# baegwangbin/MaGNet

Measured on NVIDIA H100. Metric: frames/sec (640x480, 4 views, 64 hyp), higher is better.
Workload: dtype f32

## Files before the change

magnet_b200/csrc/cost_mma.cu:

```cuda
#include <cuda_bf16.h>
#include <cuda_fp16.h>

#include <algorithm>
#include <atomic>
#include <cstddef>
#include <mutex>
#include <type_traits>

#include "common.cuh"
#include "tma_common.cuh"
#include "cw_mask.cuh"

namespace magnet {

constexpr int MNT = 256;
constexpr int MTW = 8, MTH = 8;
constexpr int MPX = MTW * MTH;
constexpr int MCH = 64;
constexpr int MSEG = 32;
constexpr int MMAXV = 16;
constexpr int SEG_BYTES = 2048;
constexpr int META_SEG_BYTES = 128;
constexpr uint32_t SEG_TX = 1024;
constexpr uint32_t REF_TX = 8192;

constexpr int MOFF_A = 0;
constexpr int MOFF_R = 16384;
constexpr int MR_BYTES = 67584;
constexpr int MOFF_META = MOFF_R + MR_BYTES;
constexpr int MOFF_CAM = MOFF_META + MSEG * META_SEG_BYTES;
constexpr int MOFF_KS = MOFF_CAM + MMAXV * 64;
constexpr int MOFF_BBOX = MOFF_KS + MCH * 4;
constexpr int MOFF_BAR = MOFF_BBOX + 64;
constexpr int MOFF_DV = MOFF_BAR + 64;
constexpr int MOFF_DEND = MOFF_DV + MPX * 65 * 4;
constexpr int MOFF_PIXR = MOFF_DEND + MPX * 8;
constexpr int MOFF_PIX = MOFF_PIXR + MPX * 32;
constexpr int M_SMEM_USED = MOFF_PIX + 8 * 8 * 32;
constexpr int M_SMEM_TOTAL = M_SMEM_USED + 1024;
static_assert(MR_BYTES >= MSEG * SEG_BYTES && MR_BYTES >= MPX * 264 * 4 && MR_BYTES >= MCH * 65 * 4, "region R");
constexpr int MMA_DBG_OUTSIDE = 16 + MPX * 256;
static_assert(2 * (M_SMEM_TOTAL + 1024) <= 227 * 1024, "two CTAs per SM");

__host__ __device__ inline size_t split16_bytes(size_t N, size_t H, size_t W) {
  return SPLIT16_HEADER + N * H * W * 256 + N * H * (W + 1) * 16;
}
__host__ __device__ inline size_t half16_bytes(size_t N, size_t H, size_t W) {
  return SPLIT16_HEADER + N * H * W * 128 + N * H * (W + 1) * 16;
}

constexpr int MMA_SLOTS = 1024;
__device__ unsigned g_mma_next[MMA_SLOTS];
__device__ unsigned g_mma_done[MMA_SLOTS];

__device__ __forceinline__ float lds_f32(uint32_t a) {
  float v;
  asm volatile("ld.shared.f32 %0, [%1];" : "=f"(v) : "r"(a));
  return v;
}
__device__ __forceinline__ float4 lds_f32x4(uint32_t a) {
  float4 v;
  asm volatile("ld.shared.v4.f32 {%0, %1, %2, %3}, [%4];" : "=f"(v.x), "=f"(v.y), "=f"(v.z), "=f"(v.w) : "r"(a));
  return v;
}
enum { PROF_SETUP, PROF_BOX, PROF_TMA, PROF_MMA, PROF_PHASEC, PROF_EPI, PROF_NSTAGES };
#ifdef MAGNET_MMA_PROFILE
#define MMA_STAGE(s)                                                                                                   \
  do {                                                                                                                 \
    if (tid == 0) {                                                                                                    \
      const long long t_ = clock64();                                                                                  \
      prof_s[s] += t_ - prof_s[7];                                                                                     \
      prof_s[7] = t_;                                                                                                  \
    }                                                                                                                  \
  } while (0)
#else
#define MMA_STAGE(s) do { } while (0)
#endif

template <int MODE, bool CW, int PLANES>
__global__ void __launch_bounds__(MNT, 2)
cost_mma_kernel(const __grid_constant__ CostParams p, const __grid_constant__ CUtensorMap tm_ref,
                const __grid_constant__ CUtensorMap tm_src, const __grid_constant__ CUtensorMap tm_meta, const int nchunks,
                const int n_items, const int slot, float* __restrict__ dbg) {
  extern __shared__ unsigned char smem_raw[];
  const uint32_t raw = smem_u32(smem_raw);
  const uint32_t padb = (1024u - (raw & 1023u)) & 1023u;
  unsigned char* smem = smem_raw + padb;
  const uint32_t sbase = raw + padb;
  const magnet_camera* cams_s = reinterpret_cast<const magnet_camera*>(smem + MOFF_CAM);
  float* ks = reinterpret_cast<float*>(smem + MOFF_KS);
  int* bbox = reinterpret_cast<int*>(smem + MOFF_BBOX);
  float* regR = reinterpret_cast<float*>(smem + MOFF_R);
  const uint32_t bar_tma = sbase + MOFF_BAR, bar_cam = sbase + MOFF_BAR + 24;
  const unsigned FULL = 0xffffffffu;

  const int tid = threadIdx.x, lane = tid & 31, warp = tid >> 5;
#ifdef MAGNET_MMA_PROFILE
  __shared__ long long prof_s[8];
  if (tid < 8) prof_s[tid] = tid == 7 ? clock64() : 0ll;
#endif
  const int H = p.H, W = p.W, HW = p.HW, D = p.D, V = p.V;
  const int tiles_x = (W + MTW - 1) / MTW;
  const int items_per_b = tiles_x * ((H + MTH - 1) / MTH) * nchunks;

  const unsigned char* refbuf = reinterpret_cast<const unsigned char*>(p.ref_feat);
  const unsigned char* srcbuf = reinterpret_cast<const unsigned char*>(p.src_feat);
  const Split16Header* hdr_ref = reinterpret_cast<const Split16Header*>(refbuf);
  const Split16Header* hdr_src = reinterpret_cast<const Split16Header*>(srcbuf);
  volatile int* next_item = reinterpret_cast<volatile int*>(smem + MOFF_BAR + 40);

  if (tid == 0) {
    mbar_init(bar_tma, 1);
    mbar_init(bar_cam, 1);
    fence_mbar_init();
    prefetch_tmap(&tm_ref);
    prefetch_tmap(&tm_src);
    prefetch_tmap(&tm_meta);
  }
  if (tid < 8) bbox[tid] = (tid & 1) ? -(1 << 28) : (1 << 28);
  __syncthreads();
  uint32_t ph_tma = 0, ph_cam = 0;
  int it = 0;
  int cur_b = -1;
  const float xmax = (float)W + 1.0f, ymax = (float)H + 1.0f;
  const float kappa = p.kappa;
  constexpr float BOX_EPS = 0.015625f;
  const float amp_max = 65536.0f / (float)(max(W, H) + 3) - 8.0f;
  const uint32_t g_row0 = sbase + MOFF_R, m_base = sbase + MOFF_META;

  int item = blockIdx.x;
  while (item < n_items) {
  const int b = item / items_per_b;
  const int rem = item - b * items_per_b;
  const int tile = rem / nchunks;
  const int jc = (rem - tile * nchunks) * MCH;
  const int Dc = min(MCH, D - jc);
  const int tx0 = (tile % tiles_x) * MTW, ty0 = (tile / tiles_x) * MTH;

  if (tid == 0) {
    if (b != cur_b) {
      mbar_arrive_expect_tx(bar_cam, (uint32_t)V * 64u);
      bulk_load(sbase + MOFF_CAM, p.cams + (size_t)b * V, (uint32_t)V * 64u, bar_cam);
    }
    tma_load_5d(sbase + MOFF_A, &tm_ref, bar_tma, 0, tx0, ty0, 0, b);
    *next_item = (int)gridDim.x + (int)atomicAdd(&g_mma_next[slot], 1u);
  }
  if (tid < MCH) ks[tid] = MODE != MAGNET_DEPTH_VOLUME ? p.k[min(jc + tid, D - 1)] : 0.0f;
  __syncthreads();

  const int py = ty0 + warp;
  float4* pixr = reinterpret_cast<float4*>(smem + MOFF_PIXR) + warp * 16;
  unsigned livemask;
  {
    float R0, R1, R2, MU = 0.f, SG = 0.f;
    const int px = tx0 + (lane & 7);
    const bool live = px < W && py < H;
    const int n = min(py, H - 1) * W + min(px, W - 1);
    R0 = ldg_f(p.rays + ((size_t)b * 3 + 0) * HW + n);
    R1 = ldg_f(p.rays + ((size_t)b * 3 + 1) * HW + n);
    R2 = ldg_f(p.rays + ((size_t)b * 3 + 2) * HW + n);
    if (MODE == MAGNET_DEPTH_GAUSS) {
      MU = ldg_f(p.ref_gmm + ((size_t)b * 2 + 0) * HW + n);
      SG = ldg_f(p.ref_gmm + ((size_t)b * 2 + 1) * HW + n);
    }
    livemask = __ballot_sync(FULL, live) & 0xffu;
    if (lane < 8) {
      pixr[2 * lane] = make_float4(R0, R1, R2, 0.0f);
      pixr[2 * lane + 1] = make_float4(MU, SG, 0.0f, 0.0f);
    }
    __syncwarp();
  }
  const uint32_t dvw = sbase + MOFF_DV + (uint32_t)(warp * 8 * 65 + lane) * 4u;
  if (MODE == MAGNET_DEPTH_VOLUME) {
    float* dv_s = reinterpret_cast<float*>(smem + MOFF_DV);
    const int pp = tid & 63, y = ty0 + (pp >> 3), x = tx0 + (pp & 7);
    const float* dsrc = p.d_volume + ((size_t)b * D + jc) * HW + (size_t)min(y, H - 1) * W + min(x, W - 1);
#pragma unroll 1
    for (int j0 = tid >> 6; j0 < MCH; j0 += 32) {
      float dl[8];
#pragma unroll
      for (int r = 0; r < 8; ++r) dl[r] = ldg_f(dsrc + (size_t)min(j0 + 4 * r, Dc - 1) * HW);
#pragma unroll
      for (int r = 0; r < 8; ++r) dv_s[pp * 65 + j0 + 4 * r] = dl[r];
    }
    __syncthreads();
#pragma unroll
    for (int i = 0; i < MTW; ++i) {
      const float da = lds_f32(dvw + i * 260), db = lds_f32(dvw + i * 260 + 128);
      float lo = fminf(da, db), hi = fmaxf(da, db);
      const bool fin = __all_sync(FULL, isfinite(da) && isfinite(db));
#pragma unroll
      for (int o = 16; o > 0; o >>= 1) {
        lo = fminf(lo, __shfl_xor_sync(FULL, lo, o));
        hi = fmaxf(hi, __shfl_xor_sync(FULL, hi, o));
      }
      if (lane == i) reinterpret_cast<float2*>(smem + MOFF_DEND)[warp * 8 + i] = fin ? make_float2(lo, hi) : make_float2(NAN, NAN);
    }
    __syncwarp();
  }
  auto depth2 = [&](const int i, const float mu, const float sg) -> float2 {
    if (MODE == MAGNET_DEPTH_VOLUME) return make_float2(lds_f32(dvw + i * 260), lds_f32(dvw + i * 260 + 128));
    const float2 k2 = make_float2(ks[lane], ks[lane + 32]);
    if (MODE == MAGNET_DEPTH_PLANES) return k2;
    return fadd2_rn(make_float2(mu, mu), make_float2(__fmul_rn(sg, k2.x), __fmul_rn(sg, k2.y)));
  };
  float4* pixt = reinterpret_cast<float4*>(smem + MOFF_PIX) + warp * 16;

  auto window_box = [&](const int v, int* bb) {
    const magnet_camera* cam = cams_s + v;
    const float a0 = cam->a[0], a1 = cam->a[1], a2 = cam->a[2];
    const float4 ray = pixr[2 * (lane & 7)];
    const float MU = pixr[2 * (lane & 7) + 1].x, SG = pixr[2 * (lane & 7) + 1].y;
    const float Q0 = __fmaf_rn(cam->A[2], ray.z, __fmaf_rn(cam->A[1], ray.y, __fmul_rn(cam->A[0], ray.x)));
    const float Q1 = __fmaf_rn(cam->A[5], ray.z, __fmaf_rn(cam->A[4], ray.y, __fmul_rn(cam->A[3], ray.x)));
    const float Q2 = __fmaf_rn(cam->A[8], ray.z, __fmaf_rn(cam->A[7], ray.y, __fmul_rn(cam->A[6], ray.x)));
    float2 dr;
    if (MODE == MAGNET_DEPTH_VOLUME) {
      const uint32_t a = sbase + MOFF_DEND + (uint32_t)(warp * 8 + (lane & 7)) * 8u;
      dr = make_float2(lds_f32(a), lds_f32(a + 4));
    }
    else if (MODE == MAGNET_DEPTH_PLANES) dr = make_float2(ks[0], ks[MCH - 1]);
    else dr = fadd2_rn(make_float2(MU, MU), make_float2(__fmul_rn(SG, ks[0]), __fmul_rn(SG, ks[MCH - 1])));
    float2 ix, iy, z;
    project2(dr, a0, a1, a2, Q0, Q1, Q2, ix, iy, z);
    const float amp = fmaxf(fabsf(__fmul_rn(Q2, dr.x)) / z.x, fabsf(__fmul_rn(Q2, dr.y)) / z.y) + 2.0e-3f / fminf(z.x, z.y);
    const bool ok = (MODE == MAGNET_DEPTH_VOLUME || p.k_sorted) && isfinite(dr.x) && isfinite(dr.y) && z.x > 0.0f &&
                    z.y > 0.0f && amp <= amp_max && isfinite(ix.x) && isfinite(ix.y) && isfinite(iy.x) && isfinite(iy.y);
    const bool live = (livemask >> (lane & 7)) & 1u;
    float xl = 1e9f, xh = -1e9f, yl = 1e9f, yh = -1e9f;
    if (__all_sync(FULL, ok || !live)) {
      if (live) {
        xl = clamp_coord(__fsub_rn(fminf(ix.x, ix.y), BOX_EPS), xmax); xh = clamp_coord(__fadd_rn(fmaxf(ix.x, ix.y), BOX_EPS), xmax);
        yl = clamp_coord(__fsub_rn(fminf(iy.x, iy.y), BOX_EPS), ymax); yh = clamp_coord(__fadd_rn(fmaxf(iy.x, iy.y), BOX_EPS), ymax);
      }
    } else {
#ifdef MAGNET_MMA_DEBUG
      if (dbg != nullptr && lane == 0) atomicAdd(reinterpret_cast<unsigned*>(dbg + MMA_DBG_OUTSIDE + 1), 1u);
#endif
#pragma unroll
      for (int i = 0; i < MTW; ++i) {
        const float q0 = __shfl_sync(FULL, Q0, i), q1 = __shfl_sync(FULL, Q1, i), q2 = __shfl_sync(FULL, Q2, i);
        const float mu = __shfl_sync(FULL, MU, i), sg = __shfl_sync(FULL, SG, i);
        project2(depth2(i, mu, sg), a0, a1, a2, q0, q1, q2, ix, iy, z);
        ix.x = clamp_coord(ix.x, xmax); ix.y = clamp_coord(ix.y, xmax);
        iy.x = clamp_coord(iy.x, ymax); iy.y = clamp_coord(iy.y, ymax);
        if ((livemask >> i) & 1u) {
          xl = fminf(xl, fminf(ix.x, ix.y)); xh = fmaxf(xh, fmaxf(ix.x, ix.y));
          yl = fminf(yl, fminf(iy.x, iy.y)); yh = fmaxf(yh, fmaxf(iy.x, iy.y));
        }
      }
    }
    const int r0 = __reduce_min_sync(FULL, (int)floorf(xl)), r1 = __reduce_max_sync(FULL, (int)floorf(xh));
    const int r2 = __reduce_min_sync(FULL, (int)floorf(yl)), r3 = __reduce_max_sync(FULL, (int)floorf(yh));
    if (lane == 0) { atomicMin(bb + 0, r0); atomicMax(bb + 1, r1); atomicMin(bb + 2, r2); atomicMax(bb + 3, r3); }
  };
  auto next_valid = [&](int v) {
    while (v < V && cams_s[v].valid != 1.0f) ++v;
    return v;
  };

  if (b != cur_b) {
    mbar_wait_or_trap(bar_cam, ph_cam);
    ph_cam ^= 1u;
    cur_b = b;
  }
  bool first = true;
  float2 accr[MTW];
#pragma unroll
  for (int i = 0; i < MTW; ++i) accr[i] = make_float2(0.0f, 0.0f);
  MMA_STAGE(PROF_SETUP);
  int v = next_valid(0);
  if (v < V) window_box(v, bbox + (it & 1) * 4);
  __syncthreads();
  MMA_STAGE(PROF_BOX);

  while (v < V) {
    const int vn = next_valid(v + 1);
    __syncwarp();
    if (lane < 8) {
      const magnet_camera* cam = cams_s + v;
      const float4 ray = pixr[2 * lane], ms = pixr[2 * lane + 1];
      const float Q0 = __fmaf_rn(cam->A[2], ray.z, __fmaf_rn(cam->A[1], ray.y, __fmul_rn(cam->A[0], ray.x)));
      const float Q1 = __fmaf_rn(cam->A[5], ray.z, __fmaf_rn(cam->A[4], ray.y, __fmul_rn(cam->A[3], ray.x)));
      const float Q2 = __fmaf_rn(cam->A[8], ray.z, __fmaf_rn(cam->A[7], ray.y, __fmul_rn(cam->A[6], ray.x)));
      pixt[2 * lane] = make_float4(Q0, Q1, Q2, cam->a[0]);
      pixt[2 * lane + 1] = make_float4(cam->a[1], ms.x, ms.y, cam->a[2]);
    }
    __syncwarp();
    const int vb = v * p.B + b;
    auto project_px = [&](const int i, float2& ix, float2& iy, float2& z) {
      const float4 t1 = pixt[2 * i], t2 = pixt[2 * i + 1];
      project2(depth2(i, t2.y, t2.z), t1.w, t2.x, t2.w, t1.x, t1.y, t1.z, ix, iy, z);
      ix.x = clamp_coord(ix.x, xmax); ix.y = clamp_coord(ix.y, xmax);
      iy.x = clamp_coord(iy.x, ymax); iy.y = clamp_coord(iy.y, ymax);
    };

    const int* bb = bbox + (it & 1) * 4;
    const int wx0 = bb[0], wx1 = bb[1], wy0 = bb[2], wy1 = bb[3];
    ++it;
    const int nseg_all = (wx1 - wx0 + 2 + 7) >> 3, rows_all = wy1 - wy0 + 2;
    const int nsw = min(nseg_all, 16);
    const int rmax = nseg_all * rows_all <= MSEG ? rows_all : max(2, MSEG / nsw);
    const int stepx = 8 * nsw - 1, stepy = rmax - 1;

    for (int sy = wy0; sy <= wy1; sy += stepy) {
      const int rows = min(stepy, wy1 - sy + 1) + 1;
      for (int sx = wx0; sx <= wx1; sx += stepx) {
        const int nseg = (min(stepx, wx1 - sx + 1) + 1 + 7) >> 3;
        const int nsegs = nseg * rows;
        if (tid == 0)
          mbar_arrive_expect_tx(bar_tma, (uint32_t)nsegs * (SEG_TX * PLANES + (CW ? META_SEG_BYTES : 0)) + (first ? REF_TX * PLANES : 0u));
        first = false;
        if (lane == 0) {
          for (int s = warp; s < nsegs; s += MNT / 32) {
            const int r = s / nseg, xb = s - r * nseg;
            tma_load_5d(sbase + MOFF_R + (uint32_t)s * SEG_BYTES, &tm_src, bar_tma, 0, sx + 8 * xb, sy + r, 0, vb);
            if (CW) tma_load_4d(m_base + (uint32_t)s * META_SEG_BYTES, &tm_meta, bar_tma, 0, sx + 8 * xb + 1, sy + r, vb);
          }
        }
        __syncwarp();
        const bool first_pass = sy == wy0 && sx == wx0;
        if (first_pass && vn < V) window_box(vn, bbox + (it & 1) * 4);
        const int npad = (nsegs * 8 + 15) & ~15;
        const int gp = ((npad + 23) & ~31) + 8;
        mbar_wait_or_trap(bar_tma, ph_tma);
        ph_tma ^= 1u;
        MMA_STAGE(PROF_TMA);
        {
          const int wg = warp >> 2;
          float acc[64];
#pragma unroll
          for (int e = 0; e < 64; ++e) acc[e] = 0.0f;
          const uint32_t bseg = sbase + MOFF_R + (uint32_t)(wg * 16 * SEG_BYTES);
          const uint64_t a_hi = gmma_desc_sw128(sbase + MOFF_A, 1024), a_lo = gmma_desc_sw128(sbase + MOFF_A + 8192, 1024);
          const uint64_t b_hi = gmma_desc_sw128(bseg, SEG_BYTES), b_lo = gmma_desc_sw128(bseg + 1024, SEG_BYTES);
          __syncwarp();
          constexpr bool WG1_N64 = (CW || MODE != MAGNET_DEPTH_GAUSS) && (PLANES == 2 || CW || MODE != MAGNET_DEPTH_VOLUME);
          if (wg == 0 || npad > (WG1_N64 ? 192 : 128)) {
            wgmma_fence();
#pragma unroll
            for (int pr = PLANES == 2 ? 0 : 2; pr < 3; ++pr) {
              const uint64_t ad = pr == 0 ? a_lo : a_hi, bd = pr == 1 ? b_lo : b_hi;
#pragma unroll
              for (int kk = 0; kk < 4; ++kk) wgmma_m64n128k16_f16(acc, ad + 2u * kk, bd + 2u * kk, ((PLANES == 2 ? pr : 0) | kk) != 0);
            }
            wgmma_commit();
            wgmma_wait_all();
          } else if (WG1_N64 && npad > 128) {
            float (&acc64)[32] = *reinterpret_cast<float (*)[32]>(acc);
            wgmma_fence();
#pragma unroll
            for (int pr = PLANES == 2 ? 0 : 2; pr < 3; ++pr) {
              const uint64_t ad = pr == 0 ? a_lo : a_hi, bd = pr == 1 ? b_lo : b_hi;
#pragma unroll
              for (int kk = 0; kk < 4; ++kk) wgmma_m64n64k16_f16(acc64, ad + 2u * kk, bd + 2u * kk, ((PLANES == 2 ? pr : 0) | kk) != 0);
            }
            wgmma_commit();
            wgmma_wait_all();
          }
          __syncthreads();
          if (tid == 0 && first_pass) *reinterpret_cast<int4*>(bbox + ((it + 1) & 1) * 4) = make_int4(1 << 28, -(1 << 28), 1 << 28, -(1 << 28));
          const int r0 = ((warp & 3) << 4) + (lane >> 2);
          float* g0 = regR + (size_t)r0 * gp + wg * 128 + 2 * (lane & 3);
#pragma unroll
          for (int j = 0; j < 16; ++j) {
            if (wg * 128 + 8 * j < npad) {
              *reinterpret_cast<float2*>(g0 + 8 * j) = make_float2(acc[4 * j], acc[4 * j + 1]);
              *reinterpret_cast<float2*>(g0 + 8 * gp + 8 * j) = make_float2(acc[4 * j + 2], acc[4 * j + 3]);
            }
          }
          __syncthreads();
        }
        MMA_STAGE(PROF_MMA);
#ifdef MAGNET_MMA_DEBUG
        if (dbg != nullptr && item == 0 && v == 0 && sy == wy0 && sx == wx0) {
          if (tid == 0) {
            dbg[0] = (float)sx; dbg[1] = (float)sy; dbg[2] = (float)nseg; dbg[3] = (float)rows; dbg[4] = (float)npad;
            dbg[5] = (float)gp; dbg[6] = (float)v; dbg[7] = 2.0f * PLANES - 1.0f; dbg[8] = hdr_ref->scale; dbg[9] = hdr_src->scale;
          }
          for (int idx = tid; idx < MPX * npad; idx += MNT) dbg[16 + (idx / npad) * 256 + idx % npad] = regR[(idx / npad) * gp + idx % npad];
        }
#endif
        const bool single = nseg_all * rows_all <= MSEG;
        auto phase_c = [&](auto single_tag) {
          constexpr bool SINGLE = decltype(single_tag)::value;
          const float MAGIC = 12582912.0f;
          const float sxf = (float)sx, syf = (float)sy;
          const float xend = sx + stepx > wx1 ? 1e9f : (float)(sx + stepx), yend = sy + stepy > wy1 ? 1e9f : (float)(sy + stepy);
          const float pitch4f = (float)(nseg * 32);
          const float c0f = MAGIC - 4.0f * sxf - pitch4f * syf;
          const uint32_t pitch4 = (uint32_t)nseg * 32u;
          uint32_t rowaddr = g_row0 + (uint32_t)(warp * 8 * gp) * 4u;
          const uint32_t cmax = pitch4 * (uint32_t)(rows - 1) - 8u;
#pragma unroll
          for (int i = 0; i < MTW; ++i, rowaddr += (uint32_t)gp * 4u) {
            if (!((livemask >> i) & 1u)) continue;
            float2 x, y, z;
            project_px(i, x, y, z);
            float2 x0, y0, fx, fy;
            cell_split(x.x, x0.x, fx.x); cell_split(x.y, x0.y, fx.y);
            cell_split(y.x, y0.x, fy.x); cell_split(y.y, y0.y, fy.y);
            const float2 m1 = make_float2(-1.0f, -1.0f);
            const float2 o = ffma2_rn(y0, make_float2(pitch4f, pitch4f), ffma2_rn(x0, make_float2(4.0f, 4.0f), make_float2(c0f, c0f)));
            uint32_t ca = __float_as_uint(o.x) & 0x3fffffu, cb = __float_as_uint(o.y) & 0x3fffffu;
            bool pa = true, pb = true;
            if (!SINGLE) {
              pa = x0.x >= sxf && x0.x < xend && y0.x >= syf && y0.x < yend;
              pb = x0.y >= sxf && x0.y < xend && y0.y >= syf && y0.y < yend;
              ca = pa ? ca : 0u;
              cb = pb ? cb : 0u;
            } else {
              ca = min(ca, cmax);
              cb = min(cb, cmax);
            }
#ifdef MAGNET_MMA_DEBUG
            if (dbg != nullptr && sy == wy0 && sx == wx0) {
              const bool outa = lane < Dc && (x0.x < (float)wx0 || x0.x > (float)wx1 || y0.x < (float)wy0 || y0.x > (float)wy1);
              const bool outb = lane + 32 < Dc && (x0.y < (float)wx0 || x0.y > (float)wx1 || y0.y < (float)wy0 || y0.y > (float)wy1);
              const unsigned nout = __popc(__ballot_sync(FULL, outa)) + __popc(__ballot_sync(FULL, outb));
              if (lane == 0 && nout != 0u) atomicAdd(reinterpret_cast<unsigned*>(dbg + MMA_DBG_OUTSIDE), nout);
            }
#endif
            const uint32_t ga = rowaddr + ca, gb = rowaddr + cb;
            const float2 g00 = make_float2(lds_f32(ga), lds_f32(gb)), g01 = make_float2(lds_f32(ga + 4), lds_f32(gb + 4));
            const float2 g10 = make_float2(lds_f32(ga + pitch4), lds_f32(gb + pitch4));
            const float2 g11 = make_float2(lds_f32(ga + pitch4 + 4), lds_f32(gb + pitch4 + 4));
            const float2 ct = ffma2_rn(fx, ffma2_rn(g00, m1, g01), g00), cu = ffma2_rn(fx, ffma2_rn(g10, m1, g11), g10);
            const float2 cost = ffma2_rn(fy, ffma2_rn(ct, m1, cu), ct);
            const float costa = cost.x, costb = cost.y;
            bool oka, okb;
            if (CW) {
              const uint32_t ma = m_base + ca * 4u, mb = m_base + cb * 4u;
              const float2 msa = lerp2d_x2(lds_f32x4(ma), lds_f32x4(ma + pitch4 * 4u), fx.x, fy.x);
              const float2 msb = lerp2d_x2(lds_f32x4(mb), lds_f32x4(mb + pitch4 * 4u), fx.y, fy.y);
              oka = cw_keep(z.x, msa, kappa);
              okb = cw_keep(z.y, msb, kappa);
            } else {
              oka = fabsf(costa) < 3.0e38f;
              okb = fabsf(costb) < 3.0e38f;
            }
            if (pa && oka) accr[i].x += costa;
            if (pb && okb) accr[i].y += costb;
          }
        };
        if (single) phase_c(std::true_type{});
        else phase_c(std::false_type{});
        fence_proxy_async();
        __syncthreads();
        MMA_STAGE(PROF_PHASEC);
      }
    }
    v = vn;
  }

  if (first) {
    if (tid == 0) mbar_arrive_expect_tx(bar_tma, REF_TX * PLANES);
    mbar_wait_or_trap(bar_tma, ph_tma);
    ph_tma ^= 1u;
  }

  {
    float* acc_s = regR;
    const int b = item / items_per_b;
    const int rem = item - b * items_per_b;
    const int tile = rem / nchunks;
    const int jc = (rem - tile * nchunks) * MCH;
    const int Dc = min(MCH, D - jc);
    const int tx0 = (tile % tiles_x) * MTW, ty0 = (tile / tiles_x) * MTH;
#pragma unroll
    for (int i = 0; i < MTW; ++i) {
      acc_s[lane * 65 + warp * 8 + i] = accr[i].x;
      acc_s[(lane + 32) * 65 + warp * 8 + i] = accr[i].y;
    }
    __syncthreads();
    const float inv = hdr_ref->inv_scale * hdr_src->inv_scale;
    const bool exact = p.inv_v_exact != 0.0f;
    auto fin = [&](float a) { a *= inv; return exact ? a * p.inv_v_exact : __fdiv_rn(a, p.vf); };
    if ((W & 3) == 0 && (reinterpret_cast<uintptr_t>(p.out) & 15) == 0) {
      for (int idx = tid; idx < MCH * 16; idx += MNT) {
        const int j = idx >> 4, r = (idx >> 1) & 7, hx = (idx & 1) * 4;
        const int y = ty0 + r, x = tx0 + hx;
        if (j < Dc && x < W && y < H) {
          const float* a = acc_s + j * 65 + r * 8 + hx;
          *reinterpret_cast<float4*>(p.out + ((size_t)b * D + jc + j) * HW + (size_t)y * W + x) =
              make_float4(fin(a[0]), fin(a[1]), fin(a[2]), fin(a[3]));
        }
      }
    } else {
      for (int idx = tid; idx < MCH * MPX; idx += MNT) {
        const int j = idx >> 6, pp = idx & 63;
        const int y = ty0 + (pp >> 3), x = tx0 + (pp & 7);
        if (j < Dc && x < W && y < H) p.out[((size_t)b * D + jc + j) * HW + (size_t)y * W + x] = fin(acc_s[j * 65 + pp]);
      }
    }
  }
  const int nxt = *next_item;
  fence_proxy_async();
  __syncthreads();
  MMA_STAGE(PROF_EPI);
  item = nxt;
  }

#ifdef MAGNET_MMA_PROFILE
  if (tid == 0 && dbg != nullptr) {
    unsigned long long* tot = reinterpret_cast<unsigned long long*>(dbg);
    for (int s = 0; s < PROF_NSTAGES; ++s) atomicAdd(tot + s, (unsigned long long)prof_s[s]);
    atomicAdd(tot + 7, 1ull);
  }
#endif
  if (tid == 0) {
    __threadfence();
    if (atomicAdd(&g_mma_done[slot], 1u) == gridDim.x - 1) {
      g_mma_next[slot] = 0u;
      g_mma_done[slot] = 0u;
      __threadfence();
    }
  }
}

__device__ __forceinline__ unsigned finite_abs_bits(float x) {
  const unsigned u = __float_as_uint(x) & 0x7fffffffu;
  return u >= 0x7f800000u ? 0u : u;
}
__device__ __forceinline__ float to_f32(float x) { return x; }
__device__ __forceinline__ float to_f32(__half x) { return __half2float(x); }
__device__ __forceinline__ float to_f32(__nv_bfloat16 x) { return __bfloat162float(x); }

template <class T>
__global__ void __launch_bounds__(256) absmax_kernel(const T* __restrict__ x, size_t n16, const T* __restrict__ tail,
                                                     int ntail, unsigned* __restrict__ out) {
  unsigned m = 0u;
  for (size_t i = (size_t)blockIdx.x * blockDim.x + threadIdx.x; i < n16; i += (size_t)gridDim.x * blockDim.x) {
    if constexpr (std::is_same<T, float>::value) {
      const float4 v = __ldg(reinterpret_cast<const float4*>(x) + i);
      m = max(max(m, finite_abs_bits(v.x)), finite_abs_bits(v.y));
      m = max(max(m, finite_abs_bits(v.z)), finite_abs_bits(v.w));
    } else {
      const uint4 r = __ldg(reinterpret_cast<const uint4*>(x) + i);
      const T* h = reinterpret_cast<const T*>(&r);
#pragma unroll
      for (int e = 0; e < 8; ++e) m = max(m, finite_abs_bits(to_f32(h[e])));
    }
  }
  if (blockIdx.x == 0 && (int)threadIdx.x < ntail) m = max(m, finite_abs_bits(to_f32(tail[threadIdx.x])));
  m = __reduce_max_sync(0xffffffffu, m);
  if ((threadIdx.x & 31) == 0 && m != 0u) atomicMax(out, m);
}

template <class T> __device__ __forceinline__ float4 ldg_x4(const T* p) {
  if constexpr (std::is_same<T, float>::value) {
    return __ldg(reinterpret_cast<const float4*>(p));
  } else {
    const uint2 r = __ldg(reinterpret_cast<const uint2*>(p));
    const T* h = reinterpret_cast<const T*>(&r);
    return make_float4(to_f32(h[0]), to_f32(h[1]), to_f32(h[2]), to_f32(h[3]));
  }
}

template <class T, int PLANES, int SPX, bool VEC>
__global__ void __launch_bounds__(256) split16_repack_kernel(const T* __restrict__ src, const float* __restrict__ gmm,
                                                             unsigned char* __restrict__ dst, int N, int HW, int W) {
  constexpr int C = 64;
  __shared__ float t[SPX * (C + 1)];
  Split16Header* hdr = reinterpret_cast<Split16Header*>(dst);
  const int sh = split16_shift(hdr->absmax);
  const float s = __uint_as_float((unsigned)(127 + sh) << 23);
  if (blockIdx.x == 0 && blockIdx.y == 0 && threadIdx.x == 0) {
    hdr->scale = s;
    hdr->inv_scale = __uint_as_float((unsigned)(127 - sh) << 23);
  }
  const size_t img = blockIdx.y;
  const int p0 = blockIdx.x * SPX;
  if constexpr (VEC) {
    static_assert(SPX == 128, "thread mapping below");
    constexpr int CPI = 8;
    const int lane = threadIdx.x & 31, warp = threadIdx.x >> 5;
    const int q4 = (warp & 3) * 8 + (lane & 7), c0 = (warp >> 2) * 4 + (lane >> 3);
    float4 v[C / CPI];
#pragma unroll
    for (int e = 0; e < C / CPI; ++e) {
      const int c = c0 + e * CPI, pix = p0 + 4 * q4;
      v[e] = pix < HW ? ldg_x4(src + (img * C + c) * HW + pix) : make_float4(0.f, 0.f, 0.f, 0.f);
    }
#pragma unroll
    for (int e = 0; e < C / CPI; ++e) {
      const int c = c0 + e * CPI;
      t[(4 * q4 + 0) * (C + 1) + c] = v[e].x;
      t[(4 * q4 + 1) * (C + 1) + c] = v[e].y;
      t[(4 * q4 + 2) * (C + 1) + c] = v[e].z;
      t[(4 * q4 + 3) * (C + 1) + c] = v[e].w;
    }
  } else {
    const int xi = threadIdx.x % SPX, cy = threadIdx.x / SPX;
    for (int c = cy; c < C; c += 256 / SPX) t[xi * (C + 1) + c] = p0 + xi < HW ? to_f32(src[(img * C + c) * HW + p0 + xi]) : 0.0f;
  }
  __syncthreads();
  __half* planes = reinterpret_cast<__half*>(dst + SPLIT16_HEADER);
  float4* meta = reinterpret_cast<float4*>(dst + SPLIT16_HEADER + (size_t)N * HW * 128 * PLANES);
#pragma unroll
  for (int itw = 0; itw < SPX * 8 / 256; ++itw) {
    const int item = itw * 256 + threadIdx.x;
    const int pl = item >> 3, q = item & 7;
    if (p0 + pl < HW) {
      __align__(16) __half hi[8], lo[8];
#pragma unroll
      for (int e = 0; e < 8; ++e) {
        const float v = t[pl * (C + 1) + q * 8 + e] * s;
        hi[e] = __float2half_rn(v);
        if constexpr (PLANES == 2) lo[e] = __float2half_rn(v - __half2float(hi[e]));
      }
      const size_t o = (size_t)(p0 + pl) * 64 + q * 8;
      *reinterpret_cast<uint4*>(planes + (img * PLANES + 0) * (size_t)HW * 64 + o) = *reinterpret_cast<const uint4*>(hi);
      if constexpr (PLANES == 2)
        *reinterpret_cast<uint4*>(planes + (img * 2 + 1) * (size_t)HW * 64 + o) = *reinterpret_cast<const uint4*>(lo);
    }
  }
  if (threadIdx.x < SPX && p0 + threadIdx.x < HW) {
    const int pix = p0 + threadIdx.x;
    const int y = pix / W, x = pix - y * W;
    float2 ms = make_float2(0.0f, 0.0f);
    if (gmm != nullptr) ms = make_float2(gmm[(img * 2 + 0) * HW + pix], gmm[(img * 2 + 1) * HW + pix]);
    float2* row = reinterpret_cast<float2*>(meta + (img * (HW / W) + y) * (size_t)(W + 1));
    row[2 * (x + 1)] = ms;
    row[2 * x + 1] = ms;
    if (x == 0) row[0] = make_float2(0.0f, 0.0f);
    if (x == W - 1) row[2 * W + 1] = make_float2(0.0f, 0.0f);
  }
}

int sm_count(int dev) {
  static int cached[64] = {0};
  int& c = cached[dev & 63];
  if (c == 0) {
    int n = 0;
    if (cudaDeviceGetAttribute(&n, cudaDevAttrMultiProcessorCount, dev) != cudaSuccess || n <= 0) n = 132;
    c = n;
  }
  return c;
}

template <class T>
static cudaError_t launch_repack_planes(const T* src, const float* gmm, void* dst, int N, int C, int H, int W,
                                       cudaStream_t st, int* launches) {
  constexpr int PLANES = std::is_same<T, float>::value ? 2 : 1;
  constexpr size_t VEC = 16 / sizeof(T);
  if (C != 64) return cudaErrorInvalidValue;
  const int HW = H * W;
  const size_t n = (size_t)N * C * HW;
  cudaError_t e = cudaMemsetAsync(dst, 0, SPLIT16_HEADER, st);
  if (e != cudaSuccess) return e;
  const size_t n16 = n / VEC;
  int dev = 0;
  if ((e = cudaGetDevice(&dev)) != cudaSuccess) return e;
  const int blocks = (int)std::min<size_t>((size_t)sm_count(dev) * 8, (n16 + 255) / 256 + 1);
  absmax_kernel<T><<<blocks, 256, 0, st>>>(src, n16, src + n16 * VEC, (int)(n - n16 * VEC),
                                           reinterpret_cast<unsigned*>(static_cast<unsigned char*>(dst) + offsetof(Split16Header, absmax)));
  dim3 block(256);
  if (HW % 4 == 0 && reinterpret_cast<uintptr_t>(src) % 16 == 0) {
    dim3 grid((HW + 127) / 128, N);
    split16_repack_kernel<T, PLANES, 128, true><<<grid, block, 0, st>>>(src, gmm, static_cast<unsigned char*>(dst), N, HW, W);
  } else {
    dim3 grid((HW + 31) / 32, N);
    split16_repack_kernel<T, PLANES, 32, false><<<grid, block, 0, st>>>(src, gmm, static_cast<unsigned char*>(dst), N, HW, W);
  }
  *launches = 2;
  return cudaGetLastError();
}

cudaError_t launch_absmax_f32(const float* x, size_t n, unsigned* out, cudaStream_t st) {
  cudaError_t e = cudaMemsetAsync(out, 0, sizeof(unsigned), st);
  if (e != cudaSuccess) return e;
  int dev = 0;
  if ((e = cudaGetDevice(&dev)) != cudaSuccess) return e;
  const size_t n16 = n / 4;
  const int blocks = (int)std::min<size_t>((size_t)sm_count(dev) * 8, (n16 + 255) / 256 + 1);
  absmax_kernel<float><<<blocks, 256, 0, st>>>(x, n16, x + n16 * 4, (int)(n - n16 * 4), out);
  return cudaGetLastError();
}

cudaError_t launch_repack_split16(const float* src, const float* gmm, void* dst, int N, int C, int H, int W,
                                  cudaStream_t st, int* launches) {
  return launch_repack_planes(src, gmm, dst, N, C, H, W, st, launches);
}

cudaError_t launch_repack_half16(const void* src, int dtype, const float* gmm, void* dst, int N, int C, int H, int W,
                                 cudaStream_t st, int* launches) {
  if (dtype == MAGNET_DTYPE_F16)
    return launch_repack_planes(static_cast<const __half*>(src), gmm, dst, N, C, H, W, st, launches);
  return launch_repack_planes(static_cast<const __nv_bfloat16*>(src), gmm, dst, N, C, H, W, st, launches);
}

typedef CUresult (*EncodeTiledFn)(CUtensorMap*, CUtensorMapDataType, cuuint32_t, void*, const cuuint64_t*,
                                  const cuuint64_t*, const cuuint32_t*, const cuuint32_t*, CUtensorMapInterleave,
                                  CUtensorMapSwizzle, CUtensorMapL2promotion, CUtensorMapFloatOOBfill);
EncodeTiledFn encode_tiled_fn();

cudaError_t make_planes_map(CUtensorMap* tm, const void* planes, int N, int H, int W, int box_rows, int nplanes) {
  EncodeTiledFn enc = encode_tiled_fn();
  if (!enc) return cudaErrorNotSupported;
  const cuuint64_t dims[5] = {64, (cuuint64_t)W, (cuuint64_t)H, (cuuint64_t)nplanes, (cuuint64_t)N};
  const cuuint64_t strides[4] = {128, (cuuint64_t)W * 128, (cuuint64_t)H * W * 128, (cuuint64_t)H * W * 128 * nplanes};
  const cuuint32_t box[5] = {64u, 8u, (cuuint32_t)box_rows, (cuuint32_t)nplanes, 1u};
  const cuuint32_t estr[5] = {1u, 1u, 1u, 1u, 1u};
  const CUresult r = enc(tm, CU_TENSOR_MAP_DATA_TYPE_FLOAT16, 5, const_cast<void*>(planes), dims, strides, box, estr,
                         CU_TENSOR_MAP_INTERLEAVE_NONE, CU_TENSOR_MAP_SWIZZLE_128B, CU_TENSOR_MAP_L2_PROMOTION_L2_256B,
                         CU_TENSOR_MAP_FLOAT_OOB_FILL_NONE);
  return r == CUDA_SUCCESS ? cudaSuccess : cudaErrorInvalidValue;
}

static cudaError_t make_meta_map(CUtensorMap* tm, const void* meta, int N, int H, int W) {
  EncodeTiledFn enc = encode_tiled_fn();
  if (!enc) return cudaErrorNotSupported;
  const cuuint64_t dims[4] = {4, (cuuint64_t)W + 1, (cuuint64_t)H, (cuuint64_t)N};
  const cuuint64_t strides[3] = {16, ((cuuint64_t)W + 1) * 16, (cuuint64_t)H * (W + 1) * 16};
  const cuuint32_t box[4] = {4u, 8u, 1u, 1u};
  const cuuint32_t estr[4] = {1u, 1u, 1u, 1u};
  const CUresult r = enc(tm, CU_TENSOR_MAP_DATA_TYPE_FLOAT32, 4, const_cast<void*>(meta), dims, strides, box, estr,
                         CU_TENSOR_MAP_INTERLEAVE_NONE, CU_TENSOR_MAP_SWIZZLE_NONE, CU_TENSOR_MAP_L2_PROMOTION_L2_128B,
                         CU_TENSOR_MAP_FLOAT_OOB_FILL_NONE);
  return r == CUDA_SUCCESS ? cudaSuccess : cudaErrorInvalidValue;
}

#if defined(MAGNET_MMA_DEBUG) || defined(MAGNET_MMA_PROFILE)
static float* g_mma_dbg = nullptr;
void mma_set_debug_buffer(float* p) { g_mma_dbg = p; }
#endif

template <int MODE, bool CW, int PLANES>
static cudaError_t launch_mma_mw(const CostParams& p, cudaStream_t st) {
  static std::once_flag flags[64];
  auto kern = cost_mma_kernel<MODE, CW, PLANES>;
  int dev = 0;
  cudaError_t e = cudaGetDevice(&dev);
  if (e != cudaSuccess) return e;
  cudaError_t res = cudaSuccess;
  std::call_once(flags[dev & 63], [&] {
    res = cudaFuncSetAttribute(kern, cudaFuncAttributeMaxDynamicSharedMemorySize, M_SMEM_TOTAL);
    if (res == cudaSuccess)
      res = cudaFuncSetAttribute(kern, cudaFuncAttributePreferredSharedMemoryCarveout, cudaSharedmemCarveoutMaxShared);
  });
  if (res != cudaSuccess) return res;
  const int N = p.B * p.V;
  const unsigned char* refbuf = reinterpret_cast<const unsigned char*>(p.ref_feat);
  const unsigned char* srcbuf = reinterpret_cast<const unsigned char*>(p.src_feat);
  CUtensorMap tm_ref, tm_src, tm_meta;
  if ((e = make_planes_map(&tm_ref, refbuf + SPLIT16_HEADER, p.B, p.H, p.W, 8, PLANES)) != cudaSuccess) return e;
  if ((e = make_planes_map(&tm_src, srcbuf + SPLIT16_HEADER, N, p.H, p.W, 1, PLANES)) != cudaSuccess) return e;
  if ((e = make_meta_map(&tm_meta, srcbuf + SPLIT16_HEADER + (size_t)N * p.HW * 128 * PLANES, N, p.H, p.W)) != cudaSuccess)
    return e;
  const int nchunks = (p.D + MCH - 1) / MCH;
  const int tiles = ((p.W + MTW - 1) / MTW) * ((p.H + MTH - 1) / MTH);
  const int n_items = tiles * nchunks * p.B;
  static std::atomic<unsigned> ticket{0}, graph_ticket{0};
  cudaStreamCaptureStatus cap = cudaStreamCaptureStatusNone;
  if (cudaStreamIsCapturing(st, &cap) != cudaSuccess) cap = cudaStreamCaptureStatusNone;
  const int slot = cap == cudaStreamCaptureStatusActive ? MMA_SLOTS / 2 + (int)(graph_ticket.fetch_add(1) % (MMA_SLOTS / 2))
                                                        : (int)(ticket.fetch_add(1) % (MMA_SLOTS / 2));
  dim3 grid(std::min(n_items, 2 * sm_count(dev))), block(MNT);
  float* dbg = nullptr;
#if defined(MAGNET_MMA_DEBUG) || defined(MAGNET_MMA_PROFILE)
  dbg = g_mma_dbg;
#endif
  kern<<<grid, block, M_SMEM_TOTAL, st>>>(p, tm_ref, tm_src, tm_meta, nchunks, n_items, slot, dbg);
  return cudaGetLastError();
}

bool mma_supports(int C, int D, int V, int layout) {
  return C == 64 && (layout == MAGNET_SRC_SPLIT16 || layout == MAGNET_SRC_HALF16) && D >= 1 && V <= MMAXV;
}

void mma_launch_info(int B, int H, int W, int D, int* grid, int* block, int* smem) {
  int dev = 0;
  cudaGetDevice(&dev);
  *grid = std::min(((W + MTW - 1) / MTW) * ((H + MTH - 1) / MTH) * ((D + MCH - 1) / MCH) * B, 2 * sm_count(dev));
  *block = MNT;
  *smem = M_SMEM_TOTAL;
}

size_t split16_buffer_bytes(int N, int H, int W) { return split16_bytes((size_t)N, (size_t)H, (size_t)W); }
size_t half16_buffer_bytes(int N, int H, int W) { return half16_bytes((size_t)N, (size_t)H, (size_t)W); }

template <int PLANES>
static cudaError_t launch_cost_mma_planes(const CostParams& p, int mode, bool cw, cudaStream_t st) {
  if (cw) {
    if (mode == MAGNET_DEPTH_VOLUME) return launch_mma_mw<MAGNET_DEPTH_VOLUME, true, PLANES>(p, st);
    if (mode == MAGNET_DEPTH_GAUSS) return launch_mma_mw<MAGNET_DEPTH_GAUSS, true, PLANES>(p, st);
    return launch_mma_mw<MAGNET_DEPTH_PLANES, true, PLANES>(p, st);
  }
  if (mode == MAGNET_DEPTH_VOLUME) return launch_mma_mw<MAGNET_DEPTH_VOLUME, false, PLANES>(p, st);
  if (mode == MAGNET_DEPTH_GAUSS) return launch_mma_mw<MAGNET_DEPTH_GAUSS, false, PLANES>(p, st);
  return launch_mma_mw<MAGNET_DEPTH_PLANES, false, PLANES>(p, st);
}

cudaError_t launch_cost_mma(const CostParams& p, int mode, bool cw, int layout, cudaStream_t st) {
  if (layout == MAGNET_SRC_HALF16) return launch_cost_mma_planes<1>(p, mode, cw, st);
  return launch_cost_mma_planes<2>(p, mode, cw, st);
}

}
```

Measured before the change: 6971.

## Fuse absmax header finalize into last block, drop memsets, stream repack loads

Result: faster. 7318, median of 6 (+5.0%).

```diff
diff --git a/magnet_b200/csrc/cost_mma.cu b/magnet_b200/csrc/cost_mma.cu
--- a/magnet_b200/csrc/cost_mma.cu
+++ b/magnet_b200/csrc/cost_mma.cu
@@ -526,32 +526,80 @@
 __device__ __forceinline__ float to_f32(__half x) { return __half2float(x); }
 __device__ __forceinline__ float to_f32(__nv_bfloat16 x) { return __bfloat162float(x); }
 
-template <class T>
+template <class T> __device__ __forceinline__ unsigned finite_abs_bits16(uint4 r) {
+  const T* h = reinterpret_cast<const T*>(&r);
+  unsigned m = 0u;
+#pragma unroll
+  for (int e = 0; e < (int)(16 / sizeof(T)); ++e) m = max(m, finite_abs_bits(to_f32(h[e])));
+  return m;
+}
+
+constexpr int ABSMAX_SLOTS = 1024;
+__device__ unsigned g_absmax_max[ABSMAX_SLOTS];
+__device__ unsigned g_absmax_done[ABSMAX_SLOTS];
+
+static int absmax_slot(cudaStream_t st) {
+  static std::atomic<unsigned> ticket{0}, graph_ticket{0};
+  cudaStreamCaptureStatus cap = cudaStreamCaptureStatusNone;
+  if (cudaStreamIsCapturing(st, &cap) != cudaSuccess) cap = cudaStreamCaptureStatusNone;
+  return cap == cudaStreamCaptureStatusActive ? ABSMAX_SLOTS / 2 + (int)(graph_ticket.fetch_add(1) % (ABSMAX_SLOTS / 2))
+                                              : (int)(ticket.fetch_add(1) % (ABSMAX_SLOTS / 2));
+}
+
+template <class T, bool HEADER>
 __global__ void __launch_bounds__(256) absmax_kernel(const T* __restrict__ x, size_t n16, const T* __restrict__ tail,
-                                                     int ntail, unsigned* __restrict__ out) {
+                                                     int ntail, unsigned* __restrict__ out, int slot) {
+  constexpr int U = 4;
+  __shared__ unsigned red[8];
+  __shared__ bool last;
+  const uint4* v = reinterpret_cast<const uint4*>(x);
+  const size_t stride = (size_t)gridDim.x * blockDim.x;
+  size_t i = (size_t)blockIdx.x * blockDim.x + threadIdx.x;
   unsigned m = 0u;
-  for (size_t i = (size_t)blockIdx.x * blockDim.x + threadIdx.x; i < n16; i += (size_t)gridDim.x * blockDim.x) {
-    if constexpr (std::is_same<T, float>::value) {
-      const float4 v = __ldg(reinterpret_cast<const float4*>(x) + i);
-      m = max(max(m, finite_abs_bits(v.x)), finite_abs_bits(v.y));
-      m = max(max(m, finite_abs_bits(v.z)), finite_abs_bits(v.w));
-    } else {
-      const uint4 r = __ldg(reinterpret_cast<const uint4*>(x) + i);
-      const T* h = reinterpret_cast<const T*>(&r);
-#pragma unroll
-      for (int e = 0; e < 8; ++e) m = max(m, finite_abs_bits(to_f32(h[e])));
-    }
-  }
+  for (; i + (U - 1) * stride < n16; i += U * stride) {
+    uint4 r[U];
+#pragma unroll
+    for (int u = 0; u < U; ++u) r[u] = __ldg(v + i + u * stride);
+#pragma unroll
+    for (int u = 0; u < U; ++u) m = max(m, finite_abs_bits16<T>(r[u]));
+  }
+  for (; i < n16; i += stride) m = max(m, finite_abs_bits16<T>(__ldg(v + i)));
   if (blockIdx.x == 0 && (int)threadIdx.x < ntail) m = max(m, finite_abs_bits(to_f32(tail[threadIdx.x])));
   m = __reduce_max_sync(0xffffffffu, m);
-  if ((threadIdx.x & 31) == 0 && m != 0u) atomicMax(out, m);
+  if ((threadIdx.x & 31) == 0) red[threadIdx.x >> 5] = m;
+  __syncthreads();
+  if (threadIdx.x == 0) {
+    for (int w = 1; w < 8; ++w) m = max(m, red[w]);
+    if (m != 0u) atomicMax(&g_absmax_max[slot], m);
+    __threadfence();
+    last = atomicAdd(&g_absmax_done[slot], 1u) == gridDim.x - 1;
+  }
+  __syncthreads();
+  if (!last) return;
+  if (threadIdx.x == 0) {
+    __threadfence();
+    red[0] = atomicExch(&g_absmax_max[slot], 0u);
+    g_absmax_done[slot] = 0u;
+  }
+  __syncthreads();
+  m = red[0];
+  if constexpr (HEADER) {
+    static_assert(sizeof(Split16Header) == 12 && SPLIT16_HEADER == 256, "header words below");
+    const int sh = split16_shift(m);
+    const unsigned word = threadIdx.x == 0 ? (unsigned)(127 + sh) << 23
+                        : threadIdx.x == 1 ? (unsigned)(127 - sh) << 23
+                        : threadIdx.x == 2 ? m : 0u;
+    if (threadIdx.x < SPLIT16_HEADER / 4) out[threadIdx.x] = word;
+  } else if (threadIdx.x == 0) {
+    *out = m;
+  }
 }
 
 template <class T> __device__ __forceinline__ float4 ldg_x4(const T* p) {
   if constexpr (std::is_same<T, float>::value) {
-    return __ldg(reinterpret_cast<const float4*>(p));
+    return __ldcs(reinterpret_cast<const float4*>(p));
   } else {
-    const uint2 r = __ldg(reinterpret_cast<const uint2*>(p));
+    const uint2 r = __ldcs(reinterpret_cast<const uint2*>(p));
     const T* h = reinterpret_cast<const T*>(&r);
     return make_float4(to_f32(h[0]), to_f32(h[1]), to_f32(h[2]), to_f32(h[3]));
   }
@@ -562,15 +610,9 @@
                                                              unsigned char* __restrict__ dst, int N, int HW, int W) {
   constexpr int C = 64;
   __shared__ float t[SPX * (C + 1)];
-  Split16Header* hdr = reinterpret_cast<Split16Header*>(dst);
-  const int sh = split16_shift(hdr->absmax);
-  const float s = __uint_as_float((unsigned)(127 + sh) << 23);
-  if (blockIdx.x == 0 && blockIdx.y == 0 && threadIdx.x == 0) {
-    hdr->scale = s;
-    hdr->inv_scale = __uint_as_float((unsigned)(127 - sh) << 23);
-  }
-  const size_t img = blockIdx.y;
-  const int p0 = blockIdx.x * SPX;
+  const float s = reinterpret_cast<const Split16Header*>(dst)->scale;
+  const size_t img = gridDim.y - 1 - blockIdx.y;
+  const int p0 = (gridDim.x - 1 - blockIdx.x) * SPX;
   if constexpr (VEC) {
     static_assert(SPX == 128, "thread mapping below");
     constexpr int CPI = 8;
@@ -610,9 +652,9 @@
         if constexpr (PLANES == 2) lo[e] = __float2half_rn(v - __half2float(hi[e]));
       }
       const size_t o = (size_t)(p0 + pl) * 64 + q * 8;
-      *reinterpret_cast<uint4*>(planes + (img * PLANES + 0) * (size_t)HW * 64 + o) = *reinterpret_cast<const uint4*>(hi);
+      __stcs(reinterpret_cast<uint4*>(planes + (img * PLANES + 0) * (size_t)HW * 64 + o), *reinterpret_cast<const uint4*>(hi));
       if constexpr (PLANES == 2)
-        *reinterpret_cast<uint4*>(planes + (img * 2 + 1) * (size_t)HW * 64 + o) = *reinterpret_cast<const uint4*>(lo);
+        __stcs(reinterpret_cast<uint4*>(planes + (img * 2 + 1) * (size_t)HW * 64 + o), *reinterpret_cast<const uint4*>(lo));
     }
   }
   if (threadIdx.x < SPX && p0 + threadIdx.x < HW) {
@@ -647,14 +689,13 @@
   if (C != 64) return cudaErrorInvalidValue;
   const int HW = H * W;
   const size_t n = (size_t)N * C * HW;
-  cudaError_t e = cudaMemsetAsync(dst, 0, SPLIT16_HEADER, st);
-  if (e != cudaSuccess) return e;
   const size_t n16 = n / VEC;
   int dev = 0;
-  if ((e = cudaGetDevice(&dev)) != cudaSuccess) return e;
+  cudaError_t e = cudaGetDevice(&dev);
+  if (e != cudaSuccess) return e;
   const int blocks = (int)std::min<size_t>((size_t)sm_count(dev) * 8, (n16 + 255) / 256 + 1);
-  absmax_kernel<T><<<blocks, 256, 0, st>>>(src, n16, src + n16 * VEC, (int)(n - n16 * VEC),
-                                           reinterpret_cast<unsigned*>(static_cast<unsigned char*>(dst) + offsetof(Split16Header, absmax)));
+  absmax_kernel<T, true><<<blocks, 256, 0, st>>>(src, n16, src + n16 * VEC, (int)(n - n16 * VEC),
+                                                 static_cast<unsigned*>(dst), absmax_slot(st));
   dim3 block(256);
   if (HW % 4 == 0 && reinterpret_cast<uintptr_t>(src) % 16 == 0) {
     dim3 grid((HW + 127) / 128, N);
@@ -668,13 +709,12 @@
 }
 
 cudaError_t launch_absmax_f32(const float* x, size_t n, unsigned* out, cudaStream_t st) {
-  cudaError_t e = cudaMemsetAsync(out, 0, sizeof(unsigned), st);
+  int dev = 0;
+  cudaError_t e = cudaGetDevice(&dev);
   if (e != cudaSuccess) return e;
-  int dev = 0;
-  if ((e = cudaGetDevice(&dev)) != cudaSuccess) return e;
   const size_t n16 = n / 4;
   const int blocks = (int)std::min<size_t>((size_t)sm_count(dev) * 8, (n16 + 255) / 256 + 1);
-  absmax_kernel<float><<<blocks, 256, 0, st>>>(x, n16, x + n16 * 4, (int)(n - n16 * 4), out);
+  absmax_kernel<float, false><<<blocks, 256, 0, st>>>(x, n16, x + n16 * 4, (int)(n - n16 * 4), out, absmax_slot(st));
   return cudaGetLastError();
 }
 
```
